# eduard-permyakov/permafrost-engine

Measured on AMD Instinct MI355X. Metric: agent-steps/sec (+ flow-field cells/sec), every chunk field rebuilt + every agent stepped per tick, higher is better.
Workload: dtype u64-bitmask/u8 fields, f32 agents (f64 exp); 1 GPU; BASELINE configs[2]: 1024x1024 cells, 64 flow fields = 16384 chunk fields, 100000 agents; map_chunks=16, flow_fields=64, agents=100000, hz=20, dynamic_obstacles=0, parallelism=requests by destination + uid slabs x1, 1 all-gather (16 B/agent) per tick, ranks=1, rccl_ranks=1, backend=none, tile_exchange=auto, requests=reference planner fixture, has_dest_los=device lookup, initial_velocities=flow aligned, fields_ahead=True, tick_driver=c (navhip_tick_run), library=libnavhip.so (in-tree)

## Files before the change

permafrost-engine_amd/csrc/cohesion_kernels.hip:

```cpp
#include "navhip_internal.h"
#include "agent_internal.h"
#include "agent_thread.h"
#include "lane_group.h"

static __constant__ double c_exp2_64[64] = { NH_EXP2_64_TABLE };


#define COH_BINS 257
__global__ __launch_bounds__(256) void k_coh_plan(const int32_t *bin_start, const int32_t *flock_offsets,
                                                  const int32_t *saved, int n_flocks, int work_begin, int work_end,
                                                  int members_key, int32_t *wave_off, int32_t *perm_valid)
{
    __shared__ int32_t wsum[4];
    __shared__ int32_t carry;
    const int t = threadIdx.x, lane = t & 63, w = t >> 6;
    if(t == 0) carry = 0;
    bool same = saved[n_flocks + 1] == work_begin && saved[n_flocks + 2] == work_end && saved[n_flocks + 3] == members_key;
    for(int f = t; f <= n_flocks; f += 256) same = same && saved[f] == flock_offsets[f];
    const int valid = __syncthreads_and(same);
    for(int base = 0; base < n_flocks; base += 256) {
        const int f = base + t;
        int32_t v = 0;
        if(f < n_flocks) {
            const int32_t cnt = valid ? bin_start[(f + 1) * COH_BINS] - bin_start[f * COH_BINS]
                                      : flock_offsets[f + 1] - flock_offsets[f];
            v = (cnt + 15) >> 4;
        }
        int32_t incl = v;
#pragma unroll
        for(int d = 1; d < 64; d <<= 1) {
            int32_t o = __shfl_up(incl, d);
            if(lane >= d) incl += o;
        }
        if(lane == 63) wsum[w] = incl;
        __syncthreads();
        int32_t woff = 0;
        for(int k = 0; k < w; k++) woff += wsum[k];
        const int32_t excl = carry + woff + incl - v;
        if(f < n_flocks) wave_off[f] = excl;
        __syncthreads();
        if(t == 255) carry = excl + v;
        __syncthreads();
    }
    if(t == 0) { wave_off[n_flocks] = carry; *perm_valid = valid; }
}

__device__ __forceinline__ int coh_bin_of(const nh_step_params &P, int g, int *flock_out)
{
    int lo = 0, hi = P.n_flocks;
    while(hi - lo > 1) {
        int mid = (lo + hi) >> 1;
        if(P.flock_offsets[mid] <= g) lo = mid; else hi = mid;
    }
    *flock_out = lo;
    const int m = P.flock_members[g];
    const bool act = m >= P.work_begin && m < P.work_end && state_uses_point_seek(P.state[m])
                  && !(P.flags[m] & NAVHIP_ENTITY_FLAG_COMBAT_HELD);
    if(!act) return lo * COH_BINS + 256;
    const float ox = (float)P.grid.origin_x * (1.0f / 256.0f), oz = (float)P.grid.origin_y * (1.0f / 256.0f);
    const int bx = (int)floorf((P.pos_xz[2 * m] - ox) * (1.0f / 256.0f)) & 15;
    const int bz = (int)floorf((P.pos_xz[2 * m + 1] - oz) * (1.0f / 256.0f)) & 15;
    int mo = 0;
#pragma unroll
    for(int k = 0; k < 4; k++) mo |= (((bx >> k) & 1) << (2 * k)) | (((bz >> k) & 1) << (2 * k + 1));
    return lo * COH_BINS + mo;
}

__device__ __forceinline__ int coh_grouped_add(int32_t *counter, int bin, bool idle)
{
    const int lane = threadIdx.x & 63;
    int slot = 0;
    unsigned long long rem = __ballot(idle);
    while(rem) {
        const int leader = __ffsll((long long)rem) - 1;
        const int b0 = __shfl(bin, leader);
        const unsigned long long m = __ballot(idle && bin == b0);
        int base = 0;
        if(lane == leader) base = atomicAdd(&counter[b0], __popcll(m));
        base = __shfl(base, leader);
        if(idle && bin == b0) slot = base + __popcll(m & ((1ull << lane) - 1ull));
        rem &= ~m;
    }
    if(!idle) slot = atomicAdd(&counter[bin], 1);
    return slot;
}

__global__ __launch_bounds__(256) void k_coh_bin(nh_step_params P, int32_t *bin_of, int32_t *bin_count,
                                                 int32_t *saved)
{
    const int g = blockIdx.x * 256 + threadIdx.x;
    for(int f = g; f <= P.n_flocks; f += gridDim.x * 256) saved[f] = P.flock_offsets[f];
    if(g == 0) { saved[P.n_flocks + 1] = P.work_begin; saved[P.n_flocks + 2] = P.work_end; saved[P.n_flocks + 3] = P.members_key; }
    if(g >= P.flock_offsets[P.n_flocks]) return;
    const int m = P.flock_members[g];
    if(m < P.work_begin || m >= P.work_end) { bin_of[g] = -1; return; }
    int f;
    const int bin = coh_bin_of(P, g, &f);
    bin_of[g] = bin;
    coh_grouped_add(bin_count, bin, bin - f * COH_BINS == 256);
}

__global__ __launch_bounds__(256) void k_coh_scatter(nh_step_params P, const int32_t *bin_of,
                                                     const int32_t *bin_start, int32_t *bin_fill,
                                                     int32_t *perm)
{
    const int g = blockIdx.x * 256 + threadIdx.x;
    if(g >= P.flock_offsets[P.n_flocks]) return;
    const int bin = bin_of[g];
    if(bin < 0) return;
    perm[bin_start[bin] + coh_grouped_add(bin_fill, bin, bin % COH_BINS == 256)] = g;
}

#define COH_FAR 906.0f

#define COH_APW 16
#define COH_QS  72
#define COH_NP  2
static_assert(COH_NP % 2 == 0, "the cohesion queue is read four entries at a time: COH_NP must be even");
#define COH_G   (8 * COH_NP)

#ifdef NH_HOSTSIM
__device__ __forceinline__ float coh_keep(float x) { return x; }
#else
__device__ __forceinline__ float coh_keep(float x) { asm volatile("" : "+v"(x)); return x; }
#endif

__device__ __forceinline__ float quad_bcast(float v, int sub)
{
    switch(sub) {
    case 0:  return __int_as_float(__builtin_amdgcn_update_dpp(0, __float_as_int(v), 0x00, 0xf, 0xf, true));
    case 1:  return __int_as_float(__builtin_amdgcn_update_dpp(0, __float_as_int(v), 0x55, 0xf, 0xf, true));
    case 2:  return __int_as_float(__builtin_amdgcn_update_dpp(0, __float_as_int(v), 0xaa, 0xf, 0xf, true));
    default: return __int_as_float(__builtin_amdgcn_update_dpp(0, __float_as_int(v), 0xff, 0xf, 0xf, true));
    }
}

template <bool TAIL>
__device__ __forceinline__ void coh_batch(const float *qx, const float *qz, const double *tab, int sub,
                                          int jj, int n_valid, int self_k, v2 me, float &comx, float &comz)
{
    const f2 mex = {me.x, me.x}, mez = {me.z, me.z};
    const int lo = sub * COH_QS + (jj >> 2);
    constexpr int NP = COH_NP;
    f2 X[NP], Z[NP], ss[NP], ln[NP], tt[NP], W[NP];
    bool close = false, odd = false;
#pragma unroll
    for(int v = 0; v < NP / 2; v++) {
        const f4 xa = *(const f4*)&qx[lo + 4 * v], za = *(const f4*)&qz[lo + 4 * v];
        X[2 * v] = f2{xa.x, xa.y}; X[2 * v + 1] = f2{xa.z, xa.w};
        Z[2 * v] = f2{za.x, za.y}; Z[2 * v + 1] = f2{za.z, za.w};
    }
#pragma unroll
    for(int u = 0; u < NP; u++) {
        const f2 dx = X[u] - mex, dz = Z[u] - mez;
        ss[u] = dx * dx + dz * dz;
        f2 r = {__builtin_amdgcn_sqrtf(ss[u].x), __builtin_amdgcn_sqrtf(ss[u].y)};
        const f2 rm = {__int_as_float(__float_as_int(r.x) - 1), __int_as_float(__float_as_int(r.y) - 1)};
        const f2 rp = {__int_as_float(__float_as_int(r.x) + 1), __int_as_float(__float_as_int(r.y) + 1)};
        const f2 em = __builtin_elementwise_fma(-rm, r, ss[u]);
        const f2 ep = __builtin_elementwise_fma(-rp, r, ss[u]);
        r.x = (em.x <= 0.0f) ? rm.x : r.x;  r.y = (em.y <= 0.0f) ? rm.y : r.y;
        r.x = (ep.x > 0.0f) ? rp.x : r.x;   r.y = (ep.y > 0.0f) ? rp.y : r.y;
        ln[u] = r;
        odd |= !(ss[u].x >= 0x1p-90f && ss[u].x <= 0x1p90f) && ss[u].x != 0.0f;
        odd |= !(ss[u].y >= 0x1p-90f && ss[u].y <= 0x1p90f) && ss[u].y != 0.0f;
    }
    if(__any(odd)) {
        asm volatile("" ::: "memory");
#pragma unroll
        for(int u = 0; u < NP; u++) ln[u] = f2{__builtin_sqrtf(ss[u].x), __builtin_sqrtf(ss[u].y)};
    }
#pragma unroll
    for(int u = 0; u < NP; u++) {
        const f2 x = ln[u] - 37.5f;
        const f2 q0 = x * (1.0f / 50.0f);
        const f2 inner = __builtin_elementwise_fma(-q0, f2{50.0f, 50.0f}, x);
        tt[u] = __builtin_elementwise_fma(inner, f2{1.0f / 50.0f, 1.0f / 50.0f}, q0);
        close |= ln[u].x < 16.0f || ln[u].y < 16.0f;
    }
    if(__any(close)) {
        asm volatile("" ::: "memory");
#pragma unroll
        for(int u = 0; u < NP; u++) {
            if(ln[u].x < 16.0f) tt[u].x = cohesion_t_f64(ln[u].x);
            if(ln[u].y < 16.0f) tt[u].y = cohesion_t_f64(ln[u].y);
        }
    }
    const int k0 = jj + sub;
#pragma unroll
    for(int u = 0; u < NP; u++) {
        const f2 a = tt[u] * -6.0f;
        float w0 = exp_f32_magic(a.x, tab), w1 = exp_f32_magic(a.y, tab);
        const int ka = k0 + 8 * u, kb = ka + 4;
        if(ka == self_k || (TAIL && ka >= n_valid)) w0 = 0.0f;
        if(kb == self_k || (TAIL && kb >= n_valid)) w1 = 0.0f;
        W[u] = f2{w0, w1};
    }
#pragma unroll
    for(int u = 0; u < NP; u++) {
        const f2 px = X[u] * W[u], pz = Z[u] * W[u];
#pragma unroll
        for(int h = 0; h < 2; h++) {
            const float tx = h ? px.y : px.x, tz = h ? pz.y : pz.x;
#pragma unroll
            for(int sb = 0; sb < 4; sb++) {
                comx = coh_keep(comx + quad_bcast(tx, sb));
                comz = coh_keep(comz + quad_bcast(tz, sb));
            }
        }
    }
}

template <bool INLINE_PLAN>
__global__ __launch_bounds__(64) void k_cohesion(nh_step_params P, const int32_t *wave_off,
                                                 const int32_t *perm, const int32_t *perm_valid,
                                                 float *coh_xz, const int32_t *bin_start, const int32_t *saved)
{
    __shared__ double tab[64];
    __shared__ __attribute__((aligned(16))) float qx[4 * COH_QS];
    __shared__ __attribute__((aligned(16))) float qz[4 * COH_QS];
    const int t = threadIdx.x, sub = t & 3;
    const int wv = blockIdx.x;
    int f = 0, first_wave = 0;
    bool use_perm;
    if(INLINE_PLAN) {
        const int nf = P.n_flocks;
        bool ok = saved[nf + 1] == P.work_begin && saved[nf + 2] == P.work_end && saved[nf + 3] == P.members_key;
        if(t <= nf) ok = ok && saved[t] == P.flock_offsets[t];
        if(t == 0 && nf == 64) ok = ok && saved[64] == P.flock_offsets[64];
        use_perm = __all(ok);
        int v = 0;
        if(t < nf) {
            const int cnt = use_perm ? bin_start[(t + 1) * COH_BINS] - bin_start[t * COH_BINS]
                                     : P.flock_offsets[t + 1] - P.flock_offsets[t];
            v = (cnt + COH_APW - 1) / COH_APW;
        }
        const int incl = wave_incl_scan(v), excl = incl - v;
        if(wv >= __shfl(incl, 63)) return;
        f = __popcll(__ballot(t < nf && excl <= wv)) - 1;
        first_wave = __shfl(excl, f);
    }else{
        if(wv >= wave_off[P.n_flocks]) return;
        int lo = 0, hi = P.n_flocks;
        while(hi - lo > 1) {
            int mid = (lo + hi) >> 1;
            if(wave_off[mid] <= wv) lo = mid; else hi = mid;
        }
        f = lo;
        first_wave = wave_off[f];
        use_perm = *perm_valid != 0;
    }
    tab[t] = c_exp2_64[t];
    const float scaled_max_force = (float)((double)(0.75f / (float)P.hz) * 20.0);
    const int b = P.flock_offsets[f], e = P.flock_offsets[f + 1];
    const int pb = use_perm ? bin_start[f * COH_BINS] : b;
    const int pe = use_perm ? bin_start[(f + 1) * COH_BINS] : e;
    const int gp = pb + (wv - first_wave) * COH_APW + (t >> 2);
    const bool mine = gp < pe;
    const int g = mine ? (use_perm ? perm[gp] : gp) : -1;
    const int uid = mine ? P.flock_members[g] : -1;
    bool act = mine && uid >= P.work_begin && uid < P.work_end;
    if(act) act = state_uses_point_seek(P.state[uid]) && !(P.flags[uid] & NAVHIP_ENTITY_FLAG_COMBAT_HELD);
    if(!__syncthreads_or(act)) return;
    const v2 me = act ? mkv(P.pos_xz[2 * uid], P.pos_xz[2 * uid + 1]) : mkv(0.0f, 0.0f);
    float bx0 = act ? me.x : INFINITY, bx1 = act ? me.x : -INFINITY;
    float bz0 = act ? me.z : INFINITY, bz1 = act ? me.z : -INFINITY;
#pragma unroll
    for(int d = 4; d < 64; d <<= 1) {
        bx0 = fminf(bx0, __shfl_xor(bx0, d)); bx1 = fmaxf(bx1, __shfl_xor(bx1, d));
        bz0 = fminf(bz0, __shfl_xor(bz0, d)); bz1 = fmaxf(bz1, __shfl_xor(bz1, d));
    }
    const unsigned long long lt_mask = (1ull << t) - 1ull;
    float comx = 0.0f, comz = 0.0f;
    int self_k = -1;
    int pend = 0;
    for(int jb = b; jb < e; jb += 256) {
        int ncnt = pend;
        const int gl = act ? g - jb : -1;
#pragma unroll
        for(int q = 0; q < 4; q++) {
            const int j = jb + q * 64 + t;
            bool keep = false;
            float2 c2 = make_float2(0.0f, 0.0f);
            if(j < e) {
                const int m = P.flock_members[j];
                c2 = make_float2(P.pos_xz[2 * m], P.pos_xz[2 * m + 1]);
                const float dx = fmaxf(fmaxf(bx0 - c2.x, c2.x - bx1), 0.0f);
                const float dz = fmaxf(fmaxf(bz0 - c2.y, c2.y - bz1), 0.0f);
                keep = !(dx * dx + dz * dz > COH_FAR * COH_FAR);
            }
            const unsigned long long mk = __ballot(keep);
            const int at = ncnt + __popcll(mk & lt_mask);
            if(keep) { const int sl = (at & 3) * COH_QS + (at >> 2); qx[sl] = c2.x; qz[sl] = c2.y; }
            const int at_self = __shfl(at, gl & 63);
            if((gl >> 6) == q) self_k = at_self;
            ncnt += __popcll(mk);
        }
        const bool last = jb + 256 >= e;
        int cnt32 = ncnt & ~(COH_G - 1);
        if(last && cnt32 < ncnt) {
            const int k = ncnt + t;
            if(k < cnt32 + COH_G) { const int sl = (k & 3) * COH_QS + (k >> 2); qx[sl] = 0.0f; qz[sl] = 0.0f; }
        }
        __syncthreads();
        if(act) {
            for(int jj = 0; jj < cnt32; jj += COH_G)
                coh_batch<false>(qx, qz, tab, sub, jj, ncnt, self_k, me, comx, comz);
            if(last && cnt32 < ncnt)
                coh_batch<true>(qx, qz, tab, sub, cnt32, ncnt, self_k, me, comx, comz);
        }
        if(!last) {
            pend = ncnt - cnt32;
            float cx = 0.0f, cz = 0.0f;
            const int k = cnt32 + t;
            if(t < pend) { const int sl = (k & 3) * COH_QS + (k >> 2); cx = qx[sl]; cz = qz[sl]; }
            __syncthreads();
            if(t < pend) { const int sl = (t & 3) * COH_QS + (t >> 2); qx[sl] = cx; qz[sl] = cz; }
            self_k = (self_k >= cnt32) ? self_k - cnt32 : -1;
            __syncthreads();
        }
    }
    if(act && sub == 0) {
        const int count = (e - b) - 1;
        v2 ret = mkv(0.0f, 0.0f);
        if(count > 0) {
            const v2 cm = vscale(mkv(comx, comz), 1.0f / (float)count);
            ret = vtrunc(vsub(cm, me), scaled_max_force);
        }
        coh_xz[2 * uid] = ret.x;
        coh_xz[2 * uid + 1] = ret.z;
    }
}

struct coh_scratch {
    int32_t *wave_off, *bin_count, *bin_fill, *bin_start, *block_sum, *bin_of, *perm[2], *saved[2], *valid;
    int nb, nblocks;
};
static coh_scratch coh_layout(int32_t *scratch, int n_flocks, int n_members)
{
    coh_scratch C;
    C.nb = n_flocks * COH_BINS; C.nblocks = (C.nb + NH_SCAN_T - 1) / NH_SCAN_T;
    C.wave_off = scratch;
    C.bin_count = C.wave_off + n_flocks + 1;
    C.bin_fill = C.bin_count + C.nb;
    C.bin_start = C.bin_fill + C.nb;
    C.block_sum = C.bin_start + C.nb + 1;
    C.bin_of = C.block_sum + C.nblocks;
    C.perm[0] = C.bin_of + n_members;
    C.perm[1] = C.perm[0] + n_members;
    C.saved[0] = C.perm[1] + n_members;
    C.saved[1] = C.saved[0] + n_flocks + 4;
    C.valid = C.saved[1] + n_flocks + 4;
    return C;
}
size_t nh_cohesion_scratch_bytes(int n_flocks, int n_members)
{
    const size_t nb = (size_t)n_flocks * COH_BINS;
    return sizeof(int32_t) * (3 * ((size_t)n_flocks + 4) + 3 * nb + 1 + (nb + NH_SCAN_T - 1) / NH_SCAN_T
                              + 3 * (size_t)n_members + 1);
}

hipError_t nh_cohesion_scratch_reset(int32_t *scratch, int n_flocks, int n_members, hipStream_t s)
{
    const coh_scratch C = coh_layout(scratch, n_flocks, n_members);
    return hipMemsetAsync(C.saved[0], 0xff, sizeof(int32_t) * 2 * ((size_t)n_flocks + 4), s);
}

__global__ void k_zero_i32(int32_t *p, int n)
{
    for(int i = blockIdx.x * blockDim.x + threadIdx.x; i < n; i += gridDim.x * blockDim.x) p[i] = 0;
}

static void coh_regroup(const nh_step_params &P, const coh_scratch &C, int which, hipStream_t s)
{
    hipLaunchKernelGGL(k_zero_i32, dim3(min(64, (2 * C.nb + 255) / 256)), dim3(256), 0, s, C.bin_count, 2 * C.nb);
    const int gm = (P.n_members + 255) / 256;
    hipLaunchKernelGGL(k_coh_bin, dim3(gm), dim3(256), 0, s, P, C.bin_of, C.bin_count, C.saved[which]);
    nh_launch_scan(C.bin_count, C.bin_start, C.block_sum, C.nb, nullptr, P.grid, nullptr, s);
    hipLaunchKernelGGL(k_coh_scatter, dim3(gm), dim3(256), 0, s, P, C.bin_of, C.bin_start, C.bin_fill,
                       C.perm[which]);
}

#define COH_INLINE_PLAN_MAX 64
bool nh_launch_cohesion(const nh_step_params &P, int32_t *scratch, float *d_coh, int *parity, hipStream_t s)
{
    if(!(P.n_ents > 0 && P.n_flocks > 0 && P.n_members > 0)) return false;
    const coh_scratch C = coh_layout(scratch, P.n_flocks, P.n_members);
    const int nwaves = (P.n_members + 15) / 16 + P.n_flocks;
    const int prev = *parity ^ 1;
    if(P.n_flocks <= COH_INLINE_PLAN_MAX) {
        hipLaunchKernelGGL(k_cohesion<true>, dim3(nwaves), dim3(64), 0, s, P, (const int32_t*)C.wave_off,
                           (const int32_t*)C.perm[prev], (const int32_t*)C.valid, d_coh, (const int32_t*)C.bin_start,
                           (const int32_t*)C.saved[prev]);
        return true;
    }
    hipLaunchKernelGGL(k_coh_plan, dim3(1), dim3(256), 0, s, (const int32_t*)C.bin_start, P.flock_offsets,
                       (const int32_t*)C.saved[prev], P.n_flocks, P.work_begin, P.work_end, P.members_key, C.wave_off, C.valid);
    hipLaunchKernelGGL(k_cohesion<false>, dim3(nwaves), dim3(64), 0, s, P, (const int32_t*)C.wave_off,
                       (const int32_t*)C.perm[prev], (const int32_t*)C.valid, d_coh, (const int32_t*)C.bin_start,
                       (const int32_t*)C.saved[prev]);
    return true;
}

void nh_launch_cohesion_regroup(const nh_step_params &P, int32_t *scratch, int *parity, hipStream_t s)
{
    const coh_scratch C = coh_layout(scratch, P.n_flocks, P.n_members);
    coh_regroup(P, C, *parity, s);
    *parity ^= 1;
}
```

Measured before the change: 39.27 million agent-steps/s.

## Adaptively shrink cohesion cull radius using running sum magnitude, with verified fallback pass

After the first chunk of flock members, the cohesion kernel derives a tighter neighbour-cull radius from the magnitude of the accumulated centre-of-mass sums and the bounding box. The radius is chosen so that skipped far agents, whose exp weights are tiny, should fall below float rounding of the running sum. A running minimum of the partial sums is tracked to check that assumption, and the wave redoes the full pass with the original radius if it fails. It also pins occupancy to 8 waves per EU. The aim is to skip exp and DPP work on distant members, at the cost of extra bookkeeping and a possible second pass.

```diff
diff --git a/permafrost-engine_amd/csrc/cohesion_kernels.hip b/permafrost-engine_amd/csrc/cohesion_kernels.hip
--- a/permafrost-engine_amd/csrc/cohesion_kernels.hip
+++ b/permafrost-engine_amd/csrc/cohesion_kernels.hip
@@ -113,6 +113,27 @@
 
 #define COH_FAR 906.0f
 
+#define COH_SLACK       4
+#define COH_MARGIN      2.0f
+#define COH_WU_PER_BIT  5.78f
+__device__ __forceinline__ void coh_cull_radius(bool act, float comx, float comz, float box_max, float &R2, float &flr)
+{
+    const float ax = fabsf(comx), az = fabsf(comz);
+    const bool okl = !act || (ax >= 0x1p-100f && az >= 0x1p-100f);
+    float m = act ? fminf(ax, az) : INFINITY;
+#pragma unroll
+    for(int d = 4; d < 64; d <<= 1) m = fminf(m, __shfl_xor(m, d));
+    m = uni<64>(m);
+    if(!(__all(okl) && box_max < INFINITY)) return;
+    const int cx = ((__float_as_int(box_max + COH_FAR) >> 23) & 0xff) - 126;
+    const int em = ((__float_as_int(m) >> 23) & 0xff) - 127;
+    const int n = max(cx + 26 + COH_SLACK - em, 1);
+    const float R = 37.5f + COH_WU_PER_BIT * (float)n + COH_MARGIN;
+    if(!(R < COH_FAR)) return;
+    R2 = uni<64>(R * R);
+    flr = __int_as_float((em - COH_SLACK + 127) << 23);
+}
+
 #define COH_APW 16
 #define COH_QS  72
 #define COH_NP  2
@@ -125,6 +146,15 @@
 __device__ __forceinline__ float coh_keep(float x) { asm volatile("" : "+v"(x)); return x; }
 #endif
 
+#ifdef NH_HOSTSIM
+__device__ __forceinline__ void coh_min_abs(float &mn, float a, float b) { mn = fminf(mn, fminf(fabsf(a), fabsf(b))); }
+#else
+__device__ __forceinline__ void coh_min_abs(float &mn, float a, float b)
+{
+    asm("v_min3_f32 %0, %0, |%1|, |%2|" : "+v"(mn) : "v"(a), "v"(b));
+}
+#endif
+
 __device__ __forceinline__ float quad_bcast(float v, int sub)
 {
     switch(sub) {
@@ -137,7 +167,7 @@
 
 template <bool TAIL>
 __device__ __forceinline__ void coh_batch(const float *qx, const float *qz, const double *tab, int sub,
-                                          int jj, int n_valid, int self_k, v2 me, float &comx, float &comz)
+                                          int jj, int n_valid, int self_k, v2 me, float &comx, float &comz, float &mn)
 {
     const f2 mex = {me.x, me.x}, mez = {me.z, me.z};
     const int lo = sub * COH_QS + (jj >> 2);
@@ -206,13 +236,19 @@
             for(int sb = 0; sb < 4; sb++) {
                 comx = coh_keep(comx + quad_bcast(tx, sb));
                 comz = coh_keep(comz + quad_bcast(tz, sb));
+                coh_min_abs(mn, comx, comz);
             }
         }
     }
 }
 
+#ifdef NH_HOSTSIM
+#define COH_WAVES8
+#else
+#define COH_WAVES8 __attribute__((amdgpu_waves_per_eu(8, 8)))
+#endif
 template <bool INLINE_PLAN>
-__global__ __launch_bounds__(64) void k_cohesion(nh_step_params P, const int32_t *wave_off,
+__global__ __launch_bounds__(64) COH_WAVES8 void k_cohesion(nh_step_params P, const int32_t *wave_off,
                                                  const int32_t *perm, const int32_t *perm_valid,
                                                  float *coh_xz, const int32_t *bin_start, const int32_t *saved)
 {
@@ -270,55 +306,69 @@
         bx0 = fminf(bx0, __shfl_xor(bx0, d)); bx1 = fmaxf(bx1, __shfl_xor(bx1, d));
         bz0 = fminf(bz0, __shfl_xor(bz0, d)); bz1 = fmaxf(bz1, __shfl_xor(bz1, d));
     }
+    bx0 = uni<64>(bx0); bx1 = uni<64>(bx1); bz0 = uni<64>(bz0); bz1 = uni<64>(bz1);
+    const float box_max = uni<64>(fmaxf(fmaxf(fabsf(bx0), fabsf(bx1)), fmaxf(fabsf(bz0), fabsf(bz1))));
     const unsigned long long lt_mask = (1ull << t) - 1ull;
-    float comx = 0.0f, comz = 0.0f;
-    int self_k = -1;
-    int pend = 0;
-    for(int jb = b; jb < e; jb += 256) {
-        int ncnt = pend;
-        const int gl = act ? g - jb : -1;
-#pragma unroll
-        for(int q = 0; q < 4; q++) {
-            const int j = jb + q * 64 + t;
-            bool keep = false;
-            float2 c2 = make_float2(0.0f, 0.0f);
-            if(j < e) {
-                const int m = P.flock_members[j];
-                c2 = make_float2(P.pos_xz[2 * m], P.pos_xz[2 * m + 1]);
-                const float dx = fmaxf(fmaxf(bx0 - c2.x, c2.x - bx1), 0.0f);
-                const float dz = fmaxf(fmaxf(bz0 - c2.y, c2.y - bz1), 0.0f);
-                keep = !(dx * dx + dz * dz > COH_FAR * COH_FAR);
+    float comx, comz;
+    for(int pass = 0;; pass++) {
+        comx = 0.0f; comz = 0.0f;
+        int self_k = -1;
+        int pend = 0;
+        float flr_carry = 0.0f;
+        bool bad = false;
+        for(int jb = b; jb < e; jb += 256) {
+            float R2 = COH_FAR * COH_FAR, flr = 0.0f;
+            if(pass == 0 && jb > b) coh_cull_radius(act, comx, comz, box_max, R2, flr);
+            const float chk = uni<64>(fmaxf(flr, flr_carry));
+            float mn = fminf(fabsf(comx), fabsf(comz));
+            int ncnt = pend;
+            const int gl = act ? g - jb : -1;
+#pragma unroll
+            for(int q = 0; q < 4; q++) {
+                const int j = jb + q * 64 + t;
+                bool keep = false;
+                float2 c2 = make_float2(0.0f, 0.0f);
+                if(j < e) {
+                    const int m = P.flock_members[j];
+                    c2 = make_float2(P.pos_xz[2 * m], P.pos_xz[2 * m + 1]);
+                    const float dx = fmaxf(fmaxf(bx0 - c2.x, c2.x - bx1), 0.0f);
+                    const float dz = fmaxf(fmaxf(bz0 - c2.y, c2.y - bz1), 0.0f);
+                    keep = !(dx * dx + dz * dz > R2);
+                }
+                const unsigned long long mk = __ballot(keep);
+                const int at = ncnt + __popcll(mk & lt_mask);
+                if(keep) { const int sl = (at & 3) * COH_QS + (at >> 2); qx[sl] = c2.x; qz[sl] = c2.y; }
+                const int at_self = __shfl(at, gl & 63);
+                if((gl >> 6) == q) self_k = at_self;
+                ncnt += __popcll(mk);
             }
-            const unsigned long long mk = __ballot(keep);
-            const int at = ncnt + __popcll(mk & lt_mask);
-            if(keep) { const int sl = (at & 3) * COH_QS + (at >> 2); qx[sl] = c2.x; qz[sl] = c2.y; }
-            const int at_self = __shfl(at, gl & 63);
-            if((gl >> 6) == q) self_k = at_self;
-            ncnt += __popcll(mk);
-        }
-        const bool last = jb + 256 >= e;
-        int cnt32 = ncnt & ~(COH_G - 1);
-        if(last && cnt32 < ncnt) {
-            const int k = ncnt + t;
-            if(k < cnt32 + COH_G) { const int sl = (k & 3) * COH_QS + (k >> 2); qx[sl] = 0.0f; qz[sl] = 0.0f; }
-        }
-        __syncthreads();
-        if(act) {
-            for(int jj = 0; jj < cnt32; jj += COH_G)
-                coh_batch<false>(qx, qz, tab, sub, jj, ncnt, self_k, me, comx, comz);
-            if(last && cnt32 < ncnt)
-                coh_batch<true>(qx, qz, tab, sub, cnt32, ncnt, self_k, me, comx, comz);
-        }
-        if(!last) {
-            pend = ncnt - cnt32;
-            float cx = 0.0f, cz = 0.0f;
-            const int k = cnt32 + t;
-            if(t < pend) { const int sl = (k & 3) * COH_QS + (k >> 2); cx = qx[sl]; cz = qz[sl]; }
+            const bool last = jb + 256 >= e;
+            int cnt32 = ncnt & ~(COH_G - 1);
+            if(last && cnt32 < ncnt) {
+                const int k = ncnt + t;
+                if(k < cnt32 + COH_G) { const int sl = (k & 3) * COH_QS + (k >> 2); qx[sl] = 0.0f; qz[sl] = 0.0f; }
+            }
             __syncthreads();
-            if(t < pend) { const int sl = (t & 3) * COH_QS + (t >> 2); qx[sl] = cx; qz[sl] = cz; }
-            self_k = (self_k >= cnt32) ? self_k - cnt32 : -1;
-            __syncthreads();
-        }
+            if(act) {
+                for(int jj = 0; jj < cnt32; jj += COH_G)
+                    coh_batch<false>(qx, qz, tab, sub, jj, ncnt, self_k, me, comx, comz, mn);
+                if(last && cnt32 < ncnt)
+                    coh_batch<true>(qx, qz, tab, sub, cnt32, ncnt, self_k, me, comx, comz, mn);
+                bad |= mn < chk;
+            }
+            flr_carry = (cnt32 > 0) ? flr : chk;
+            if(!last) {
+                pend = ncnt - cnt32;
+                float cx = 0.0f, cz = 0.0f;
+                const int k = cnt32 + t;
+                if(t < pend) { const int sl = (k & 3) * COH_QS + (k >> 2); cx = qx[sl]; cz = qz[sl]; }
+                __syncthreads();
+                if(t < pend) { const int sl = (t & 3) * COH_QS + (t >> 2); qx[sl] = cx; qz[sl] = cz; }
+                self_k = (self_k >= cnt32) ? self_k - cnt32 : -1;
+                __syncthreads();
+            }
+        }
+        if(pass || !__syncthreads_or(bad)) break;
     }
     if(act && sub == 0) {
         const int count = (e - b) - 1;
```

Result: no change. 39.46 million agent-steps/s, median of 3 (+0.5%).
